# mourisl/Rcorrector

Hardware: AMD Instinct MI355X
Metric: corrected reads/sec (150 bp, k=23) (higher is better)
Workload: dtype u8/int32/u64

## Files before the change

### include/rcorrector_amd.h

```cpp
#ifndef RCORRECTOR_AMD_H
#define RCORRECTOR_AMD_H

#include <stddef.h>
#include <stdint.h>

#ifdef __cplusplus
extern "C" {
#endif

typedef struct rc_ctx rc_ctx;

typedef enum {
    RC_STATUS_OK = 0,
    RC_STATUS_ARG = -1,
    RC_STATUS_HIP = -2,
    RC_STATUS_IO = -3,
    RC_STATUS_STATE = -4,
    RC_STATUS_NOMEM = -5,
    RC_STATUS_NOSPACE = -6
} rc_status;

typedef struct {
    int device;
    int k;
// ... 124 lines not shown
    const char *qual;
    const uint32_t *off;
    char *seq2;
    const char *qual2;
    const uint32_t *off2;
    int32_t *ret, *l, *m, *h;
} rc_batch;
int rc_correct_batch(rc_ctx *ctx, rc_batch *b);

#define RC_MAX_SLOTS 4
int rc_set_slot_lanes(rc_ctx *ctx, int on);
int rc_runtime_prepare(int hw_queues);
int rc_submit(rc_ctx *ctx, const rc_batch *b, int slot);
int rc_wait(rc_ctx *ctx, int slot);
int rc_host_alloc(rc_ctx *ctx, size_t bytes, void **out);
int rc_host_free(rc_ctx *ctx, void *p);
int rc_host_register(void *p, size_t bytes);
int rc_host_unregister(void *p);

typedef struct {
    int mode;
    size_t n;
    uint64_t nbytes;
    const uint32_t *off;
    const uint32_t *bases;
    const uint8_t *qual_bits;
    const uint32_t *exc_pos;
    const uint8_t *exc_chr;
    size_t n_exc;
    int32_t *ret, *l, *m, *h;
    uint32_t *fix_pos;
    uint8_t *fix_chr;
    size_t fix_cap;
    size_t n_fix;
} rc_packed_batch;
size_t rc_pack_bases(const char *seq, size_t begin, size_t end, uint32_t *bases, uint32_t *exc_pos, uint8_t *exc_chr, size_t exc_cap);
int rc_submit_packed(rc_ctx *ctx, rc_packed_batch *b, int slot);
int rc_wait_packed(rc_ctx *ctx, int slot);
void rc_apply_fixes(char *seq, const uint32_t *fix_pos, const uint8_t *fix_chr, size_t n_fix);

typedef struct {
    int mode;
    size_t n;
    int arena_a, arena_b;
    uint64_t begin_a, bytes_a;
    uint64_t begin_b, bytes_b;
    const uint32_t *off;
    const uint8_t *qual_bits;
    int32_t *ret, *l, *m, *h;
    uint32_t *fix_pos;
    uint8_t *fix_chr;
    size_t fix_cap;
    size_t n_fix;
} rc_resident_batch;
int rc_submit_resident(rc_ctx *ctx, rc_resident_batch *b, int slot);
int rc_wait_resident(rc_ctx *ctx, int slot);

#define RC_TRACE_ITER_WORDS 36
typedef struct {
    int32_t max_iter;
    int32_t *counts_before, *counts_after;
    int32_t *flags, *n_iter;
    int32_t *iter;
} rc_trace;
int rc_correct_batch_traced(rc_ctx *ctx, rc_batch *b, rc_trace *t);

typedef struct {
    int mode;
    uint32_t n_reads;
    uint64_t nbytes;
    int32_t max_read_len;
    uint8_t *d_seq;
    const uint8_t *d_qual;
    const uint32_t *d_off;
    int32_t *d_ret, *d_l, *d_m, *d_h;
} rc_device_batch;
int rc_correct_device(rc_ctx *ctx, const rc_device_batch *b);
int rc_strong_threshold_device(rc_ctx *ctx, const uint8_t *d_seq, const uint32_t *d_off, uint32_t n_reads,
                               uint64_t nbytes, int32_t max_read_len, int32_t *d_strong);
int rc_strong_threshold_read(rc_ctx *ctx, const char *seq, int32_t *strong);
int rc_correct_read(rc_ctx *ctx, char *seq, const char *qual, int32_t pair_strong_threshold, int32_t *ret);
int rc_kmer_info_read(rc_ctx *ctx, const char *seq, int32_t *l, int32_t *m, int32_t *h);
int rc_probe_device(rc_ctx *ctx, const uint8_t *d_seq, uint64_t nbytes, int32_t *d_counts);
int rc_sync(rc_ctx *ctx);

int rc_profile_enable(rc_ctx *ctx, int on);
int rc_profile_correct_counters(rc_ctx *ctx, uint64_t *reads_listed, uint64_t *gather_rounds, uint64_t *bucket_requests);
int rc_profile_read_rounds(rc_ctx *ctx, int32_t *d_rounds);
int rc_profile_get(rc_ctx *ctx, int kernel, double *total_ms, uint64_t *launches);
int rc_profile_reset(rc_ctx *ctx);

int rc_selftest_get_bound(rc_ctx *ctx, const int32_t *c, size_t n, double error_rate, int32_t *out_int, double *out_dbl);

int rc_debug_routes(rc_ctx *ctx, uint8_t *cls_out, uint8_t *cand_out, uint64_t *runs_out, uint32_t n);

int rc_summary(const rc_ctx *ctx, uint64_t *total_reads, uint64_t *total_corrections);

#ifdef __cplusplus
}
#endif
#endif
```

### rcorrector_amd/binding.py

```python
import ctypes as C
import os
import subprocess

import numpy as np

HERE = os.path.dirname(os.path.abspath(__file__))
CSRC = os.path.join(HERE, "csrc")

ABI_SYMBOLS = [
    "rc_create", "rc_destroy", "rc_last_error", "rc_device_numa_node", "rc_device_memory",
    "rc_table_build", "rc_table_build_device", "rc_table_load_jfdump",
    "rc_table_count_begin", "rc_table_count_add", "rc_table_count_add_device", "rc_table_count_finish",
    "rc_table_count_keep", "rc_table_count_arenas", "rc_table_count_release", "rc_table_count_park", "rc_table_count_finish_sharded", "rc_submit_resident", "rc_wait_resident",
    "rc_table_count_reads_device", "rc_table_write_jfdump", "rc_table_share", "rc_table_replicate", "rc_table_replicate_async", "rc_table_lookup", "rc_table_export", "rc_table_digest", "rc_table_layout", "rc_table_stats",
    "rc_table_count_spectrum", "rc_table_spectrum",
    "rc_recount_begin", "rc_recount_add", "rc_recount_add_device", "rc_recount_follow", "rc_recount_finish",
    "rc_change_report_begin", "rc_change_report_get", "rc_change_report_end",
    "rc_weak_profile_device", "rc_weak_profile_into",
    "rc_dup_census_begin", "rc_dup_census_get", "rc_dup_census_end", "rc_read_keys_device", "rc_dup_census_merge",
    "rc_trust_profile_device", "rc_trust_profile_begin", "rc_trust_profile_get", "rc_trust_profile_end",
    "rc_mate_overlap_device", "rc_mate_overlap_begin", "rc_mate_overlap_get", "rc_mate_overlap_end",
    "rc_estimate_error_rate", "rc_bad_quality_from_hist", "rc_set_run_params", "rc_set_quality_bits", "rc_pack_quality_bits",
    "rc_correct_batch", "rc_set_slot_lanes", "rc_runtime_prepare", "rc_submit", "rc_wait", "rc_host_alloc", "rc_host_free", "rc_host_register", "rc_host_unregister", "rc_correct_batch_traced", "rc_correct_device", "rc_strong_threshold_device", "rc_probe_device", "rc_sync",
    "rc_strong_threshold_read", "rc_correct_read", "rc_kmer_info_read",
    "rc_pack_bases", "rc_submit_packed", "rc_wait_packed", "rc_apply_fixes",
    "rc_profile_enable", "rc_profile_get", "rc_profile_reset", "rc_profile_correct_counters", "rc_profile_read_rounds", "rc_selftest_get_bound", "rc_debug_routes", "rc_summary",
]


class RcorrectorError(RuntimeError):
    pass


def library_path():
    return os.environ.get("RC_LIB") or os.path.join(HERE, "librcorrector_amd.so")


def build_library(quiet=True):
    subprocess.run(["make", "-C", CSRC, "-j4", "all"], check=True,
                   stdout=subprocess.DEVNULL if quiet else None)
    return library_path()


class _Config(C.Structure):
    _fields_ = [("device", C.c_int), ("k", C.c_int), ("max_fix_per_k", C.c_int)]


class _Batch(C.Structure):
    _fields_ = [("mode", C.c_int), ("n", C.c_size_t),
                ("seq", C.c_void_p), ("qual", C.c_void_p), ("off", C.c_void_p),
                ("seq2", C.c_void_p), ("qual2", C.c_void_p), ("off2", C.c_void_p),
                ("ret", C.c_void_p), ("l", C.c_void_p), ("m", C.c_void_p), ("h", C.c_void_p)]


class _PackedBatch(C.Structure):
    _fields_ = [("mode", C.c_int), ("n", C.c_size_t), ("nbytes", C.c_uint64),
                ("off", C.c_void_p), ("bases", C.c_void_p), ("qual_bits", C.c_void_p),
                ("exc_pos", C.c_void_p), ("exc_chr", C.c_void_p), ("n_exc", C.c_size_t),
                ("ret", C.c_void_p), ("l", C.c_void_p), ("m", C.c_void_p), ("h", C.c_void_p),
                ("fix_pos", C.c_void_p), ("fix_chr", C.c_void_p), ("fix_cap", C.c_size_t), ("n_fix", C.c_size_t)]


class _ResidentBatch(C.Structure):
    _fields_ = [("mode", C.c_int), ("n", C.c_size_t), ("arena_a", C.c_int), ("arena_b", C.c_int),
                ("begin_a", C.c_uint64), ("bytes_a", C.c_uint64), ("begin_b", C.c_uint64), ("bytes_b", C.c_uint64),
                ("off", C.c_void_p), ("qual_bits", C.c_void_p),
                ("ret", C.c_void_p), ("l", C.c_void_p), ("m", C.c_void_p), ("h", C.c_void_p),
                ("fix_pos", C.c_void_p), ("fix_chr", C.c_void_p), ("fix_cap", C.c_size_t), ("n_fix", C.c_size_t)]


class _SpectrumStats(C.Structure):
    _fields_ = [("distinct", C.c_uint64), ("total", C.c_uint64), ("unique", C.c_uint64), ("max_count", C.c_uint64)]


class _RecountStats(C.Structure):
    _fields_ = [("all", _SpectrumStats), ("absent_distinct", C.c_uint64), ("absent_total", C.c_uint64)]


REPORT_MAX_LEN = 1024
REPORT_MAX_PER_READ = 64


class _ChangeReport(C.Structure):
    _fields_ = [("reads", C.c_uint64 * 2), ("reads_changed", C.c_uint64 * 2), ("reads_unfixable", C.c_uint64 * 2), ("changes", C.c_uint64 * 2),
                ("len_hist", C.c_uint64 * REPORT_MAX_LEN * 2), ("by_pos5", C.c_uint64 * REPORT_MAX_LEN * 2), ("by_pos3", C.c_uint64 * REPORT_MAX_LEN * 2),
                ("subst", C.c_uint64 * 4 * 5), ("by_qual", C.c_uint64 * 3), ("per_read", C.c_uint64 * (REPORT_MAX_PER_READ + 1))]


class _ReadWeak(C.Structure):
    _fields_ = [("weak", C.c_int32), ("bad_prefix", C.c_int32), ("bad_suffix", C.c_int32), ("uncovered", C.c_int32)]


class _DupCensus(C.Structure):
    _fields_ = [("units", C.c_uint64), ("distinct_before", C.c_uint64), ("distinct_after", C.c_uint64),
                ("copies_before", C.c_void_p), ("copies_after", C.c_void_p)]


TRUST_MAX_LEN = 1024
_TrustArray = (C.c_uint64 * TRUST_MAX_LEN) * 2
TRUST_FIELDS = ("windows", "solid5", "weak5", "solid3", "weak3")


class _TrustCounts(C.Structure):
    _fields_ = [(n, _TrustArray) for n in TRUST_FIELDS]


# ... 49 lines not shown
            "g.build()' or make -C rcorrector_amd/csrc).  There is no CPU fallback." % path)
    try:
        import torch
    except Exception:
        pass
    try:
        L = C.CDLL(path)
    except OSError as e:
        raise RcorrectorError("cannot load %s: %s" % (path, e))
    vp, sz = C.c_void_p, C.c_size_t
    L.rc_create.restype = vp
    L.rc_create.argtypes = [C.POINTER(_Config), C.c_char_p, sz]
    L.rc_destroy.argtypes = [vp]
    L.rc_last_error.restype = C.c_char_p
    L.rc_last_error.argtypes = [vp]
    L.rc_table_build.argtypes = [vp, vp, vp, sz]
    L.rc_table_build_device.argtypes = [vp, vp, vp, sz]
    L.rc_table_load_jfdump.argtypes = [vp, C.c_char_p, C.POINTER(C.c_int64)]
    L.rc_table_count_reads_device.argtypes = [vp, vp, sz, C.c_int, C.POINTER(C.c_int64)]
    L.rc_table_count_begin.argtypes = [vp]
    L.rc_table_count_add.argtypes = [vp, vp, sz]
    L.rc_table_count_add_device.argtypes = [vp, vp, sz]
    L.rc_table_count_finish.argtypes = [vp, C.c_int, C.POINTER(C.c_int64)]
    L.rc_table_count_keep.argtypes = [vp, C.c_int]
    L.rc_table_count_arenas.argtypes = [vp, C.POINTER(C.c_size_t), vp, sz]
    L.rc_table_count_release.argtypes = [vp]
    L.rc_table_count_park.argtypes = [vp]
    L.rc_table_count_finish_sharded.argtypes = [C.POINTER(C.c_void_p), C.c_int, C.c_int, C.POINTER(C.c_int64)]
    L.rc_set_slot_lanes.argtypes = [vp, C.c_int]
    if hasattr(L, "rc_runtime_prepare"):
        L.rc_runtime_prepare.argtypes = [C.c_int]
    L.rc_submit_resident.argtypes = [vp, C.POINTER(_ResidentBatch), C.c_int]
    L.rc_wait_resident.argtypes = [vp, C.c_int]
    L.rc_table_write_jfdump.argtypes = [vp, C.c_char_p, C.POINTER(C.c_int64)]
    L.rc_table_share.argtypes = [vp, vp]
    L.rc_table_replicate.argtypes = [vp, vp]
    L.rc_table_replicate_async.argtypes = [vp, vp]
    L.rc_device_numa_node.argtypes = [vp]
    L.rc_device_memory.argtypes = [vp, C.POINTER(C.c_uint64), C.POINTER(C.c_uint64)]
    L.rc_table_lookup.argtypes = [vp, vp, sz, vp]
    L.rc_table_export.argtypes = [vp, vp, vp, sz, C.POINTER(C.c_size_t)]
    L.rc_table_digest.argtypes = [vp, C.POINTER(C.c_uint64)]
    L.rc_table_layout.argtypes = [vp]
    L.rc_table_stats.argtypes = [vp, C.POINTER(C.c_uint64), C.POINTER(C.c_uint64), C.POINTER(C.c_uint64)]
    L.rc_table_count_spectrum.argtypes = [vp, C.c_uint32]
    L.rc_table_spectrum.argtypes = [vp, C.c_int, vp, C.c_uint32, C.POINTER(_SpectrumStats)]
    L.rc_recount_begin.argtypes = [vp, C.c_uint32]
    L.rc_recount_add.argtypes = [vp, vp, C.c_size_t]
    L.rc_recount_add_device.argtypes = [vp, vp, C.c_size_t]
    L.rc_recount_follow.argtypes = [vp, C.c_int]
    L.rc_recount_finish.argtypes = [vp, vp, C.POINTER(_RecountStats)]
    L.rc_change_report_begin.argtypes = [vp]
    L.rc_change_report_get.argtypes = [vp, C.POINTER(_ChangeReport)]
    L.rc_change_report_end.argtypes = [vp]
    L.rc_weak_profile_device.argtypes = [vp, vp, vp, C.c_uint32, C.c_uint64, C.c_int32, C.c_int32, vp]
    L.rc_weak_profile_into.argtypes = [vp, C.c_int, vp, C.c_int32]
    L.rc_dup_census_begin.argtypes = [vp]
    L.rc_dup_census_get.argtypes = [vp, C.c_uint32, C.POINTER(_DupCensus)]
    L.rc_dup_census_end.argtypes = [vp]
    L.rc_read_keys_device.argtypes = [vp, vp, vp, C.c_uint32, C.c_uint64, C.c_int, vp]
    L.rc_dup_census_merge.argtypes = [vp, vp]
    L.rc_trust_profile_device.argtypes = [vp, vp, vp, C.c_uint32, C.c_uint64, C.c_int32, C.c_int32, C.c_int32, vp]
    L.rc_trust_profile_begin.argtypes = [vp, C.c_int32]
    L.rc_trust_profile_get.argtypes = [vp, C.POINTER(_TrustProfile)]
    L.rc_trust_profile_end.argtypes = [vp]
    L.rc_mate_overlap_device.argtypes = [vp, vp, vp, vp, C.c_uint32, C.c_uint64, C.c_int32, C.c_int32, C.c_int32, C.c_int32, vp]
    L.rc_mate_overlap_begin.argtypes = [vp, C.c_int32, C.c_int32]
    L.rc_mate_overlap_get.argtypes = [vp, C.POINTER(_MateOverlap)]
    L.rc_mate_overlap_end.argtypes = [vp]
    L.rc_estimate_error_rate.argtypes = [vp, C.c_double, C.POINTER(C.c_double)]
    L.rc_bad_quality_from_hist.restype = C.c_char
    L.rc_bad_quality_from_hist.argtypes = [vp, vp, C.c_int32]
    L.rc_set_run_params.argtypes = [vp, C.c_double, C.c_char]
    L.rc_set_quality_bits.argtypes = [vp, C.c_int]
    L.rc_pack_quality_bits.restype = None
    L.rc_pack_quality_bits.argtypes = [vp, sz, C.c_char, vp]
    L.rc_correct_batch.argtypes = [vp, C.POINTER(_Batch)]
    L.rc_submit.argtypes = [vp, C.POINTER(_Batch), C.c_int]
    L.rc_wait.argtypes = [vp, C.c_int]
    L.rc_host_alloc.argtypes = [vp, sz, C.POINTER(C.c_void_p)]
    L.rc_host_free.argtypes = [vp, vp]
    L.rc_correct_device.argtypes = [vp, C.POINTER(_DeviceBatch)]
    L.rc_probe_device.argtypes = [vp, vp, C.c_uint64, vp]
    L.rc_strong_threshold_device.argtypes = [vp, vp, vp, C.c_uint32, C.c_uint64, C.c_int32, vp]
    L.rc_sync.argtypes = [vp]
    L.rc_strong_threshold_read.argtypes = [vp, C.c_char_p, C.POINTER(C.c_int32)]
    L.rc_correct_read.argtypes = [vp, C.c_char_p, C.c_char_p, C.c_int32, C.POINTER(C.c_int32)]
    L.rc_kmer_info_read.argtypes = [vp, C.c_char_p, C.POINTER(C.c_int32), C.POINTER(C.c_int32), C.POINTER(C.c_int32)]
    L.rc_pack_bases.restype = sz
    L.rc_pack_bases.argtypes = [vp, sz, sz, vp, vp, vp, sz]
    L.rc_submit_packed.argtypes = [vp, C.POINTER(_PackedBatch), C.c_int]
    L.rc_wait_packed.argtypes = [vp, C.c_int]
    L.rc_apply_fixes.restype = None
    L.rc_apply_fixes.argtypes = [vp, vp, vp, sz]
    L.rc_profile_enable.argtypes = [vp, C.c_int]
    L.rc_profile_get.argtypes = [vp, C.c_int, C.POINTER(C.c_double), C.POINTER(C.c_uint64)]
    L.rc_profile_reset.argtypes = [vp]
    L.rc_profile_correct_counters.argtypes = [vp, C.POINTER(C.c_uint64), C.POINTER(C.c_uint64), C.POINTER(C.c_uint64)]
    L.rc_profile_read_rounds.argtypes = [vp, vp]
    L.rc_selftest_get_bound.argtypes = [vp, vp, sz, C.c_double, vp, vp]
    L.rc_debug_routes.argtypes = [vp, vp, vp, vp, C.c_uint32]
    L.rc_summary.argtypes = [vp, C.POINTER(C.c_uint64), C.POINTER(C.c_uint64)]
    _lib = L
    return L


def runtime_prepare(hw_queues=16):
    return load_library().rc_runtime_prepare(int(hw_queues))


def pack_reads(seqs):
    lens = np.fromiter((len(s) for s in seqs), dtype=np.int64, count=len(seqs))
    off = np.zeros(len(seqs) + 1, dtype=np.uint32)
    np.cumsum(lens + 1, out=off[1:])
    if seqs:
        arena = np.frombuffer(b"\0".join(seqs) + b"\0", dtype=np.uint8).copy()
    else:
        arena = np.zeros(0, np.uint8)
    return arena, off


def unpack_reads(arena, off):
    b = arena.tobytes()
    return [b[off[i]:off[i + 1] - 1] for i in range(len(off) - 1)]


def _ptr(x):
    if x is None:
        return None
    if isinstance(x, int):
        return x
    if isinstance(x, np.ndarray):
        return x.ctypes.data
    if hasattr(x, "data_ptr"):
        if getattr(x, "is_cuda", False):
            import torch
            torch.cuda.current_stream(x.device).synchronize()
        return x.data_ptr()
    raise TypeError("cannot take a pointer of %r" % type(x))


class Context:

    def __init__(self, k=23, max_fix_per_k=4, device=0):
        self._L = load_library()
        cfg = _Config(device, k, max_fix_per_k)
        err = C.create_string_buffer(512)
        self._h = self._L.rc_create(C.byref(cfg), err, 512)
        if not self._h:
            raise RcorrectorError(err.value.decode() or "rc_create failed")
        self.k = k

    def close(self):
        if getattr(self, "_h", None):
            for p in getattr(self, "_pinned", []):
                self._L.rc_host_free(self._h, p)
            self._pinned = []
            self._L.rc_destroy(self._h)
            self._h = None

    def __del__(self):
        try:
            self.close()
        except Exception:
            pass

# ... 325 lines not shown

    def count_park(self):
        self._ck(self._L.rc_table_count_park(self._h))

    def count_finish_sharded(self, others, min_count=2):
        hs = (C.c_void_p * (1 + len(others)))(self._h, *[o._h for o in others])
        n = C.c_int64(0)
        self._ck(self._L.rc_table_count_finish_sharded(hs, 1 + len(others), min_count, C.byref(n)))
        return n.value

    def count_release(self):
        self._ck(self._L.rc_table_count_release(self._h))

    def submit_resident(self, slot, mode, off, qual_bits, arena_a, begin_a, bytes_a, arena_b=0, begin_b=0, bytes_b=0, res=None, fix_pos=None,
                        fix_chr=None, fix_cap=None):
        off = np.ascontiguousarray(off, dtype=np.uint32)
        total = len(off) - 1
        if res is None:
            res = [np.zeros(total, dtype=np.int32) for _ in range(4)]
        if fix_pos is None:
            fix_cap = int(bytes_a + bytes_b) if fix_cap is None else fix_cap
            fix_pos, fix_chr = np.zeros(fix_cap, dtype=np.uint32), np.zeros(fix_cap, dtype=np.uint8)
        b = _ResidentBatch()
        b.mode, b.n = mode, (total // 2 if mode == 1 else total)
        b.arena_a, b.begin_a, b.bytes_a = int(arena_a), int(begin_a), int(bytes_a)
        b.arena_b, b.begin_b, b.bytes_b = int(arena_b), int(begin_b), int(bytes_b)
        b.off = off.ctypes.data
        b.qual_bits = None if qual_bits is None else qual_bits.ctypes.data
        b.ret, b.l, b.m, b.h = (r.ctypes.data for r in res)
        b.fix_pos, b.fix_chr, b.fix_cap = fix_pos.ctypes.data, fix_chr.ctypes.data, len(fix_pos)
        self._ck(self._L.rc_submit_resident(self._h, C.byref(b), slot))
        if not hasattr(self, "_inflight_resident"):
            self._inflight_resident = {}
        self._inflight_resident[slot] = (b, res, fix_pos, fix_chr, (off, qual_bits))

    def wait_resident(self, slot):
        self._ck(self._L.rc_wait_resident(self._h, slot))
        b, res, fix_pos, fix_chr, _keep = self._inflight_resident.pop(slot)
        return tuple(res) + (fix_pos[:b.n_fix], fix_chr[:b.n_fix])

    def apply_fixes(self, arena, fix_pos, fix_chr):
        arena = self._arena(arena, "arena")
        fp, fc = np.ascontiguousarray(fix_pos, dtype=np.uint32), np.ascontiguousarray(fix_chr, dtype=np.uint8)
        self._L.rc_apply_fixes(arena.ctypes.data, fp.ctypes.data, fc.ctypes.data, len(fp))

    def host_array(self, n, dtype=np.uint8):
        dt = np.dtype(dtype)
        p = C.c_void_p(0)
        self._ck(self._L.rc_host_alloc(self._h, max(1, n * dt.itemsize), C.byref(p)))
        if not hasattr(self, "_pinned"):
            self._pinned = []
        self._pinned.append(p.value)
        buf = (C.c_uint8 * (n * dt.itemsize)).from_address(p.value)
        return np.frombuffer(buf, dtype=dt, count=n)


    def correct_device(self, mode, n_reads, nbytes, max_read_len, d_seq, d_qual, d_off, d_ret, d_l, d_m, d_h):
        b = _DeviceBatch(mode, n_reads, nbytes, max_read_len, _ptr(d_seq), _ptr(d_qual), _ptr(d_off),
                         _ptr(d_ret), _ptr(d_l), _ptr(d_m), _ptr(d_h))
        self._ck(self._L.rc_correct_device(self._h, C.byref(b)))

    def strong_threshold_device(self, d_seq, d_off, n_reads, nbytes, max_read_len, d_strong):
        self._ck(self._L.rc_strong_threshold_device(self._h, _ptr(d_seq), _ptr(d_off), n_reads, nbytes, max_read_len, _ptr(d_strong)))

    def strong_threshold_read(self, seq):
        out = C.c_int32(0)
        self._ck(self._L.rc_strong_threshold_read(self._h, bytes(seq), C.byref(out)))
        return out.value

    def correct_read(self, seq, qual, pair_strong_threshold=-1):
        buf = C.create_string_buffer(bytes(seq))
        out = C.c_int32(0)
        self._ck(self._L.rc_correct_read(self._h, buf, None if qual is None else bytes(qual), int(pair_strong_threshold), C.byref(out)))
        return out.value, buf.value

    def kmer_info_read(self, seq):
        l, m, h = C.c_int32(0), C.c_int32(0), C.c_int32(0)
        self._ck(self._L.rc_kmer_info_read(self._h, bytes(seq), C.byref(l), C.byref(m), C.byref(h)))
        return l.value, m.value, h.value

    def probe_device(self, d_seq, nbytes, d_counts):
        self._ck(self._L.rc_probe_device(self._h, _ptr(d_seq), nbytes, _ptr(d_counts)))

    def sync(self):
        self._ck(self._L.rc_sync(self._h))

    def profile(self, on=True):
        self._ck(self._L.rc_profile_enable(self._h, int(on)))

    def profile_correct_counters(self):
        a, b, c = C.c_uint64(0), C.c_uint64(0), C.c_uint64(0)
        self._ck(self._L.rc_profile_correct_counters(self._h, C.byref(a), C.byref(b), C.byref(c)))
        return a.value, b.value, c.value

    def profile_read_rounds(self, d_rounds=None):
        self._ck(self._L.rc_profile_read_rounds(self._h, None if d_rounds is None else d_rounds.data_ptr()))

    def profile_reset(self):
        self._ck(self._L.rc_profile_reset(self._h))

    def profile_get(self, kernel):
        ms, n = C.c_double(0), C.c_uint64(0)
        self._ck(self._L.rc_profile_get(self._h, kernel, C.byref(ms), C.byref(n)))
        return ms.value, n.value

    def selftest_get_bound(self, c, error_rate):
        c = np.ascontiguousarray(c, dtype=np.int32)
        oi = np.zeros(len(c), dtype=np.int32)
        od = np.zeros(len(c), dtype=np.float64)
        self._ck(self._L.rc_selftest_get_bound(self._h, c.ctypes.data, len(c), error_rate, oi.ctypes.data, od.ctypes.data))
        return oi, od

    def debug_routes(self, n):
        cls, cand, runs = np.zeros(n, np.uint8), np.zeros(n, np.uint8), np.zeros(n, np.uint64)
        self._ck(self._L.rc_debug_routes(self._h, cls.ctypes.data, cand.ctypes.data, runs.ctypes.data, n))
        return cls, cand, runs

    def summary(self):
        a, b = C.c_uint64(0), C.c_uint64(0)
        self._ck(self._L.rc_summary(self._h, C.byref(a), C.byref(b)))
        return a.value, b.value
```

### rcorrector_amd/csrc/rc_table.hip

```cpp
#include <cstring>
#include <vector>

#include <algorithm>
#include <vector>
#include <rocprim/rocprim.hpp>

#include <chrono>
#include "rc_internal.h"
#include "rc_device.h"

__global__ void k_home_and_index(const uint64_t *__restrict__ canon, uint32_t *__restrict__ home,
                                 uint32_t *__restrict__ idx, size_t n, uint32_t nb_home, int layout, int k, int ext)
{
    size_t j = (size_t)blockIdx.x * blockDim.x + threadIdx.x;
    if (j >= n) return;
    size_t i = n - 1 - j;
    uint32_t h, rem, xrem;
    if (layout)
        rc_packed_addr(canon[i], k, nb_home, ext, &h, &rem, &xrem);
    else
        h = rc_home(canon[i], nb_home);
    home[j] = h;
    idx[j] = (uint32_t)i;
}

__global__ void k_slot_seed(const uint32_t *__restrict__ home_sorted, long long *__restrict__ q, size_t n, int slots)
{
    size_t j = (size_t)blockIdx.x * blockDim.x + threadIdx.x;
    if (j >= n) return;
    q[j] = (long long)slots * home_sorted[j] - (long long)j;
}

__global__ void k_packed_feasible(const uint32_t *__restrict__ home_sorted, const long long *__restrict__ qmax,
                                  const int32_t *__restrict__ counts, size_t n, int ext, unsigned *__restrict__ flags)
{
    size_t j = (size_t)blockIdx.x * blockDim.x + threadIdx.x;
    if (j >= n) return;
    const long long p = qmax[j] + (long long)j;
    if ((uint32_t)counts[j] >= (RC_PACKED_COUNT_MASK >> ext)) atomicAdd(flags + 1, 1u);
    if ((uint32_t)(p / RC_PACKED_SLOTS) - home_sorted[j] > RC_PACKED_MAX_DISP) atomicOr(flags, 2u);
}

__global__ void k_collect_overflow(const uint64_t *__restrict__ canon, const int32_t *__restrict__ counts, size_t n, uint32_t cmask,
                                   unsigned *__restrict__ n_out, uint4 *__restrict__ out, uint32_t *__restrict__ out_idx)
{
    size_t i = (size_t)blockIdx.x * blockDim.x + threadIdx.x;
    if (i >= n || (uint32_t)counts[i] < cmask) return;
    const unsigned o = atomicAdd(n_out, 1u);
    if (o >= RC_PACKED_OVF_MAX) return;
    out[o] = make_uint4((uint32_t)canon[i], (uint32_t)(canon[i] >> 32), (uint32_t)counts[i], 0u);
    out_idx[o] = (uint32_t)i;
}

__global__ void k_scatter(const uint32_t *__restrict__ home_sorted, const uint32_t *__restrict__ idx_sorted,
                          const long long *__restrict__ qmax, const uint64_t *__restrict__ canon,
                          const int32_t *__restrict__ counts, uint32_t *__restrict__ buckets, size_t n, uint32_t nb_home, int layout, int k, int ext)
{
    size_t j = (size_t)blockIdx.x * blockDim.x + threadIdx.x;
    if (j >= n) return;
    const long long p = qmax[j] + (long long)j;
    const int S = rc_layout_slots(layout);
    const uint32_t b = (uint32_t)(p / S), s = (uint32_t)(p % S);
    const uint32_t i = idx_sorted[j];
    const uint64_t key = canon[i];
    if (layout) {
        uint32_t h, rem, xrem;
        rc_packed_addr(key, k, nb_home, ext, &h, &rem, &xrem);
        uint32_t *w = buckets + (size_t)b * RC_BUCKET_DWORDS + s * 2;
        w[0] = rem;
        atomicAnd(w + 1, 0x80000000u);
        const uint32_t cmask = RC_PACKED_COUNT_MASK >> ext, cnt = (uint32_t)counts[i] < cmask ? (uint32_t)counts[i] : cmask;
        atomicOr(w + 1, cnt | (xrem << (27 - ext)) | ((b - h) << 27));
        if (s == 0 && h < b) atomicOr(buckets + (size_t)(b - 1) * RC_BUCKET_DWORDS + (RC_BUCKET_DWORDS - 1), 0x80000000u);
    } else {
        uint32_t *w = buckets + (size_t)b * RC_BUCKET_DWORDS + s * 3;
        w[0] = (uint32_t)key;
        w[1] = (uint32_t)(key >> 32);
        w[2] = (uint32_t)counts[i];
        if (s == 0 && home_sorted[j] < b) buckets[(size_t)(b - 1) * RC_BUCKET_DWORDS + (RC_BUCKET_DWORDS - 1)] = 1u;
    }
}

__global__ void k_filter_set(const uint64_t *__restrict__ canon, size_t n, uint32_t nb_home, int k, int ext, uint32_t *__restrict__ filter, uint32_t words,
                             int kind)
{
    size_t i = (size_t)blockIdx.x * blockDim.x + threadIdx.x;
    if (i >= n) return;
    if (kind) {
        const uint64_t x = canon[i], rv = rc_revcomp(x, k);
        uint32_t w, m;
// ... 685 lines not shown
                const int f = (int)((w[q >> 2] >> (8 * (q & 3))) & 0xffu);
                if (i0 + q < n && f) {
#pragma unroll
                    for (int c = 0; c < NS; ++c) mine += f == first + c * step ? (1ull << (16 * c)) : 0ull;
                }
            }
        }
        uint64_t inc = mine;
#pragma unroll
        for (int o = 1; o < 64; o <<= 1) {
            const uint64_t y = __shfl_up(inc, o, 64);
            inc += lane >= (uint32_t)o ? y : 0ull;
        }
        if (lane == 63) s_wave[wave] = inc;
        __syncthreads();
        uint64_t before = 0, total = 0;
#pragma unroll
        for (int q = 0; q < 4; ++q) {
            before += (uint32_t)q < wave ? s_wave[q] : 0ull;
            total += s_wave[q];
        }
        if (total) {
            if (t < (uint32_t)NS) {
                const uint32_t c = (uint32_t)((total >> (16 * t)) & 0xffffu);
                s_base[t] = c ? atomicAdd(count + t, c) : 0u;
            }
            __syncthreads();
            if (mine) {
                const uint64_t ex = before + inc - mine;
                uint32_t pos[NS];
#pragma unroll
                for (int c = 0; c < NS; ++c) pos[c] = s_base[c] + (uint32_t)((ex >> (16 * c)) & 0xffffu);
#pragma unroll
                for (int q = 0; q < 16; ++q) {
                    const int f = (int)((w[q >> 2] >> (8 * (q & 3))) & 0xffu);
                    if (i0 + q < n && f) {
#pragma unroll
                        for (int c = 0; c < NS; ++c)
                            if (f == first + c * step) list[(size_t)c * stride + pos[c]++] = values ? values[i0 + (uint32_t)q] : i0 + (uint32_t)q;
                    }
                }
            }
        }
        __syncthreads();
    }
}

template <int NS>
static int rc_compact_sections(rc_ctx *ctx, const uint8_t *d_flag, uint32_t n, int first, int step, uint32_t *d_list, size_t stride, uint32_t *d_count,
                               const uint32_t *d_values = nullptr)
{
    RC_CHECK_HIP(ctx, hipMemsetAsync(d_count, 0, NS * sizeof(uint32_t), ctx->stream));
    if (n == 0) return RC_OK;
    unsigned grid = (n + 4095u) / 4096u;
    if (grid > (unsigned)ctx->n_cu * 32u) grid = (unsigned)ctx->n_cu * 32u;
    hipLaunchKernelGGL(k_compact_sections<NS>, dim3(grid), dim3(256), 0, ctx->stream, d_flag, n, first, step, d_list, stride, d_count, d_values);
    RC_CHECK_HIP(ctx, hipGetLastError());
    return RC_OK;
}

int rc_launch_compact(rc_ctx *ctx, const uint8_t *d_cls, uint32_t n, uint32_t *d_list, size_t stride, uint32_t *d_count)
{
    return rc_compact_sections<RC_WORK_CLASSES>(ctx, d_cls, n, RC_WORK_CLASSES, -1, d_list, stride, d_count);
}

__global__ __launch_bounds__(256) void k_gather_u8(const uint8_t *__restrict__ src, const uint32_t *__restrict__ idx, uint32_t n, uint8_t *__restrict__ dst)
{
    const uint32_t i = blockIdx.x * 256u + threadIdx.x;
    if (i < n) dst[i] = src[idx[i]];
}
int rc_launch_compact_local(rc_ctx *ctx, const uint8_t *d_cls, uint32_t n, uint32_t *d_list, size_t stride, uint32_t *d_count)
{
    int rc = rc_dbuf_reserve(ctx, &ctx->tier_flag, (size_t)n + 256);
    if (rc) return rc;
    hipLaunchKernelGGL(k_gather_u8, dim3((n + 255) / 256), dim3(256), 0, ctx->stream, d_cls, (const uint32_t *)ctx->loc_list.p, n, (uint8_t *)ctx->tier_flag.p);
    return rc_compact_sections<RC_WORK_CLASSES>(ctx, (const uint8_t *)ctx->tier_flag.p, n, RC_WORK_CLASSES, -1, d_list, stride, d_count, (const uint32_t *)ctx->loc_list.p);
}

int rc_launch_compact_flag(rc_ctx *ctx, const uint8_t *d_flag, uint32_t n, uint32_t *d_list, size_t stride, uint32_t *d_count)
{
    return rc_compact_sections<3>(ctx, d_flag, n, 1, 1, d_list, stride, d_count);
}

#define RC_KEY_TILE 40960
__global__ __launch_bounds__(256) void k_unit_key(const uint8_t *__restrict__ seq, size_t nbytes, const uint32_t *__restrict__ off,
                                                  uint32_t n_units, int mode, int k, uint32_t units_per_block,
                                                  uint32_t *__restrict__ keys, uint32_t *__restrict__ idx)
{
    __shared__ __attribute__((aligned(16))) uint8_t s_raw[RC_KEY_TILE + 48];
    const uint32_t u0 = blockIdx.x * units_per_block;
    if (u0 >= n_units) return;
    const uint32_t nu = n_units - u0 < units_per_block ? n_units - u0 : units_per_block;
    const uint32_t r0 = mode == 2 ? 2u * u0 : u0, r1 = mode == 2 ? 2u * (u0 + nu) : u0 + nu;
    const size_t b0 = off[r0], b1 = off[r1], a0 = b0 & ~(size_t)15;
    for (size_t c = threadIdx.x; a0 + 16 * c < b1; c += 256) {
        const size_t g = a0 + 16 * c;
        uint4 v = make_uint4(0, 0, 0, 0);
        if (g + 16 <= nbytes) {
            v = *reinterpret_cast<const uint4 *>(seq + g);
        } else {
            uint32_t w[4] = {0, 0, 0, 0};
            for (size_t q = 0; g + q < nbytes; ++q) w[q >> 2] |= (uint32_t)seq[g + q] << (8 * (q & 3));
            v = make_uint4(w[0], w[1], w[2], w[3]);
        }
        *reinterpret_cast<uint4 *>(s_raw + 16 * c) = v;
    }
    __syncthreads();
    if (threadIdx.x >= nu) return;
    const uint32_t u = u0 + threadIdx.x;
    const uint32_t r = mode == 2 ? 2u * u : u;
    const uint32_t o = (uint32_t)(off[r] - a0);
    const int len = (int)(off[r + 1] - off[r]) - 1;
#ifndef RC_KEY_KMER
    const int m = k < 16 ? k : 16;
    const uint32_t mask = m == 16 ? 0xFFFFFFFFu : ((1u << (2 * m)) - 1u);
    const int top = 2 * (m - 1);
    uint32_t fw = 0, rv = 0, best = 0xFFFFFFFFu;
    int valid = 0;
#ifdef RC_KEY_OFFSET
    int best_i = 0;
    bool best_rev = false;
#endif
    for (int i = 0; i < len; ++i) {
        const uint32_t c = s_raw[o + i];
        const uint32_t b = ((c >> 1) ^ (c >> 2)) & 3u;
        const uint32_t d = c - 65u;
        const bool acgt = d < 20u && ((0x80045u >> d) & 1u);
        valid = acgt ? valid + 1 : 0;
        fw = ((fw << 2) | b) & mask;
        rv = (rv >> 2) | ((3u - b) << top);
        if (valid >= m) {
            uint32_t h = (fw < rv ? fw : rv) * 0x9E3779B1u;
            h ^= h >> 15;
            h *= 0x2C1B3C6Du;
            h ^= h >> 13;
#ifdef RC_KEY_OFFSET
            if (h < best) {
                best_i = i;
                best_rev = rv < fw;
            }
#endif
            best = h < best ? h : best;
        }
    }
#ifdef RC_KEY_OFFSET
    if (best != 0xFFFFFFFFu) {
        int p = best_rev ? len - 1 - best_i : best_i - m + 1;
        p = (p >> 1) > 127 ? 127 : (p >> 1);
        best = (best & ~0x7Fu) | (uint32_t)(127 - p);
    }
#endif
#else
    const uint64_t mask = rc_kmer_mask(k);
    uint64_t fw = 0, rv = 0;
    uint32_t best = 0xFFFFFFFFu;
    int valid = 0;
    for (int i = 0; i < len; ++i) {
        const uint32_t c = s_raw[o + i];
        int b = -1;
        b = c == 'A' ? 0 : b;
        b = c == 'C' ? 1 : b;
        b = c == 'G' ? 2 : b;
        b = c == 'T' ? 3 : b;
        valid = b < 0 ? 0 : valid + 1;
        fw = ((fw << 2) | (uint64_t)(b & 3)) & mask;
        rv = (rv >> 2) | ((uint64_t)(3 - (b & 3)) << (2 * (k - 1)));
        if (valid >= k) {
            const uint32_t h = rc_hash(fw < rv ? fw : rv);
            best = h < best ? h : best;
        }
    }
#endif
    keys[u] = best;
    idx[u] = u;
}

__global__ void k_probe_order(const uint32_t *__restrict__ unit_sorted, uint32_t n, int mode, uint32_t *__restrict__ list,
                              const uint32_t *__restrict__ off, uint2 *__restrict__ span)
{
    const uint32_t i = blockIdx.x * blockDim.x + threadIdx.x;
    if (i >= n) return;
    uint32_t r;
    if (mode == 1)
        r = unit_sorted[i >> 1] + ((i & 1u) ? (n >> 1) : 0u);
    else if (mode == 2)
        r = 2u * unit_sorted[i >> 1] + (i & 1u);
    else
        r = unit_sorted[i];
    list[i] = r;
    const uint32_t g0 = off[r];
    span[i] = make_uint2(g0, off[r + 1] - g0);
}

int rc_launch_locality_order(rc_ctx *ctx, const rc_device_batch_args &a, size_t nbytes)
{
    const uint32_t n = a.n, n_units = a.mode ? n >> 1 : n;
    int rc;
    if ((rc = rc_dbuf_reserve(ctx, &ctx->loc_a, (size_t)n_units * 16 + 256))) return rc;
    if ((rc = rc_dbuf_reserve(ctx, &ctx->loc_list, (size_t)n * 4 + 256))) return rc;
    if ((rc = rc_dbuf_reserve(ctx, &ctx->loc_span, (size_t)n * 8 + 256))) return rc;
    uint32_t *keys = (uint32_t *)ctx->loc_a.p, *keys2 = keys + n_units, *idx = keys2 + n_units, *idx2 = idx + n_units;
    uint32_t upb = (uint32_t)(RC_KEY_TILE / ((size_t)(a.max_len + 1) * (a.mode == 2 ? 2 : 1)));
    if (upb > 256) upb = 256;
    if (upb < 1) upb = 1;
    hipLaunchKernelGGL(k_unit_key, dim3((n_units + upb - 1) / upb), dim3(256), 0, ctx->stream, a.seq, nbytes, a.off, n_units, a.mode, ctx->k, upb, keys, idx);
    size_t t1 = 0;
    RC_CHECK_HIP(ctx, rocprim::radix_sort_pairs(nullptr, t1, keys, keys2, idx, idx2, (size_t)n_units, 0, 32, ctx->stream));
    if ((rc = rc_dbuf_reserve(ctx, &ctx->sel_tmp, t1))) return rc;
    RC_CHECK_HIP(ctx, rocprim::radix_sort_pairs(ctx->sel_tmp.p, t1, keys, keys2, idx, idx2, (size_t)n_units, 0, 32, ctx->stream));
    hipLaunchKernelGGL(k_probe_order, dim3((n + 255) / 256), dim3(256), 0, ctx->stream, idx2, n, a.mode, (uint32_t *)ctx->loc_list.p, a.off,
                       (uint2 *)ctx->loc_span.p);
    RC_CHECK_HIP(ctx, hipGetLastError());
    return RC_OK;
}

__global__ __launch_bounds__(256) void k_tier_flags(const uint32_t *__restrict__ off, const uint32_t *__restrict__ list, uint32_t n, int mode,
                                                    int s_hi, int m_hi, uint8_t *__restrict__ flag)
{
    const uint32_t i = blockIdx.x * 256u + threadIdx.x;
    if (i >= n) return;
    const uint32_t r = list[i];
    int ml = (int)(off[r + 1] - off[r]) - 1;
    if (mode != 0) {
        const uint32_t half = n >> 1, mr = mode == 1 ? (r < half ? r + half : r - half) : (r ^ 1u);
        const int m1 = (int)(off[mr + 1] - off[mr]) - 1;
        ml = m1 > ml ? m1 : ml;
    }
    flag[i] = ml <= s_hi ? 0 : (ml <= m_hi ? 1 : 2);
}

int rc_launch_tier_lists(rc_ctx *ctx, const rc_device_batch_args &a, int s_hi, int m_hi)
{
    int rc;
    const size_t stride = ((size_t)a.n + 63) & ~(size_t)63;
    if ((rc = rc_dbuf_reserve(ctx, &ctx->tier_flag, (size_t)a.n + 256))) return rc;
    if ((rc = rc_dbuf_reserve(ctx, &ctx->tier_list, stride * 2 * 4 + 256))) return rc;
    ctx->tier_stride = stride;
    hipLaunchKernelGGL(k_tier_flags, dim3((a.n + 255) / 256), dim3(256), 0, ctx->stream, a.off, (const uint32_t *)ctx->loc_list.p, a.n, a.mode, s_hi, m_hi,
                       (uint8_t *)ctx->tier_flag.p);
    RC_CHECK_HIP(ctx, hipGetLastError());
    return rc_compact_sections<2>(ctx, (const uint8_t *)ctx->tier_flag.p, a.n, 1, 1, (uint32_t *)ctx->tier_list.p, stride,
                                  (uint32_t *)((char *)ctx->work.p + RC_WORK_NTIER_OFF), (const uint32_t *)ctx->loc_list.p);
}

template <bool EXT>
__global__ __launch_bounds__(RC_PROBE_THREADS) void k_probe(rc_table_view T, const uint8_t *__restrict__ seq,
                                                            size_t nbytes, int k, int32_t *__restrict__ counts)
{
    __shared__ uint32_t s_code[RC_PROBE_TILE / 16 + 4];
    __shared__ uint16_t s_inv[RC_PROBE_TILE / 16 + 4];
    __shared__ uint16_t s_nul[RC_PROBE_TILE / 16 + 4];
    const size_t tile0 = (size_t)blockIdx.x * RC_PROBE_TILE;
    const int t = threadIdx.x;

    rc_tile_stage(seq, 0, nbytes, tile0, s_code, s_inv, s_nul);
    __syncthreads();
    const uint32_t *m_inv = reinterpret_cast<const uint32_t *>(s_inv);
    const uint32_t *m_nul = reinterpret_cast<const uint32_t *>(s_nul);

#pragma unroll 2
    for (int a = t; a < RC_PROBE_TILE; a += RC_PROBE_THREADS) {
        const size_t g = tile0 + (size_t)a;
        if (g + (size_t)k > nbytes) break;
        const rc_tile_win w = rc_tile_window(s_code, m_inv, m_nul, a, k);
        if (w.nul) continue;
        const int cnt = w.bad ? 0 : rc_table_lookup<EXT>(T, rc_canonical(w.code, k));
        __builtin_nontemporal_store(cnt, &counts[g]);
    }
}

template <bool EXT>
__global__ __launch_bounds__(RC_PROBE_THREADS) void k_probe_list(rc_table_view T, const uint8_t *__restrict__ seq, size_t nbytes,
                                                                 const uint32_t *__restrict__ off, const uint32_t *__restrict__ list,
                                                                 uint32_t n, uint32_t reads_per_block, int k, int32_t *__restrict__ counts,
                                                                 int mode, int skip_hi, const uint32_t *__restrict__ n_list)
{
    __shared__ __attribute__((aligned(16))) uint32_t s_raw[(RC_PROBE_TILE + 64) / 4];
    __shared__ uint32_t s_code[RC_PROBE_TILE / 16 + 4];
    __shared__ uint16_t s_inv[RC_PROBE_TILE / 16 + 4];
    __shared__ uint16_t s_nul[RC_PROBE_TILE / 16 + 4];
    __shared__ uint32_t s_lpos[RC_PLIST_MAX_READS + 1], s_gpos[RC_PLIST_MAX_READS], s_len1[RC_PLIST_MAX_READS];
    const int t = threadIdx.x;
    const uint32_t n_eff = n_list ? *n_list : n;
    for (uint32_t i0 = blockIdx.x * reads_per_block; i0 < n_eff; i0 += gridDim.x * reads_per_block) {
    const uint32_t nr = n_eff - i0 < reads_per_block ? n_eff - i0 : reads_per_block;
    bool any_live = false;
    if ((uint32_t)t < nr) {
        const uint32_t r = list[i0 + t], g0 = off[r];
        uint32_t len1 = off[r + 1] - g0;
        if (skip_hi >= 0) {
            uint32_t ml1 = len1;
            if (mode != 0) {
                const uint32_t half = n >> 1, mr = mode == 1 ? (r < half ? r + half : r - half) : (r ^ 1u);
                const uint32_t m1 = off[mr + 1] - off[mr];
// ... 107 lines not shown
```

Before: 360.0 million.

## Rewrite unit-key minimizer kernel with 2-bit packed tiles and lane-parallel windows

```diff
diff --git a/include/rcorrector_amd.h b/include/rcorrector_amd.h
--- a/include/rcorrector_amd.h
+++ b/include/rcorrector_amd.h
@@ -230,6 +230,8 @@
 int rc_correct_read(rc_ctx *ctx, char *seq, const char *qual, int32_t pair_strong_threshold, int32_t *ret);
 int rc_kmer_info_read(rc_ctx *ctx, const char *seq, int32_t *l, int32_t *m, int32_t *h);
 int rc_probe_device(rc_ctx *ctx, const uint8_t *d_seq, uint64_t nbytes, int32_t *d_counts);
+int rc_unit_keys_device(rc_ctx *ctx, int mode, uint32_t n_reads, uint64_t nbytes, int32_t max_read_len, const uint8_t *d_seq,
+                        const uint32_t *d_off, uint32_t *d_keys);
 int rc_sync(rc_ctx *ctx);
 
 int rc_profile_enable(rc_ctx *ctx, int on);
diff --git a/rcorrector_amd/binding.py b/rcorrector_amd/binding.py
--- a/rcorrector_amd/binding.py
+++ b/rcorrector_amd/binding.py
@@ -21,7 +21,7 @@
     "rc_trust_profile_device", "rc_trust_profile_begin", "rc_trust_profile_get", "rc_trust_profile_end",
     "rc_mate_overlap_device", "rc_mate_overlap_begin", "rc_mate_overlap_get", "rc_mate_overlap_end",
     "rc_estimate_error_rate", "rc_bad_quality_from_hist", "rc_set_run_params", "rc_set_quality_bits", "rc_pack_quality_bits",
-    "rc_correct_batch", "rc_set_slot_lanes", "rc_runtime_prepare", "rc_submit", "rc_wait", "rc_host_alloc", "rc_host_free", "rc_host_register", "rc_host_unregister", "rc_correct_batch_traced", "rc_correct_device", "rc_strong_threshold_device", "rc_probe_device", "rc_sync",
+    "rc_correct_batch", "rc_set_slot_lanes", "rc_runtime_prepare", "rc_submit", "rc_wait", "rc_host_alloc", "rc_host_free", "rc_host_register", "rc_host_unregister", "rc_correct_batch_traced", "rc_correct_device", "rc_strong_threshold_device", "rc_probe_device", "rc_unit_keys_device", "rc_sync",
     "rc_strong_threshold_read", "rc_correct_read", "rc_kmer_info_read",
     "rc_pack_bases", "rc_submit_packed", "rc_wait_packed", "rc_apply_fixes",
     "rc_profile_enable", "rc_profile_get", "rc_profile_reset", "rc_profile_correct_counters", "rc_profile_read_rounds", "rc_selftest_get_bound", "rc_debug_routes", "rc_summary",
@@ -237,6 +237,7 @@
     L.rc_host_free.argtypes = [vp, vp]
     L.rc_correct_device.argtypes = [vp, C.POINTER(_DeviceBatch)]
     L.rc_probe_device.argtypes = [vp, vp, C.c_uint64, vp]
+    L.rc_unit_keys_device.argtypes = [vp, C.c_int, C.c_uint32, C.c_uint64, C.c_int32, vp, vp, vp]
     L.rc_strong_threshold_device.argtypes = [vp, vp, vp, C.c_uint32, C.c_uint64, C.c_int32, vp]
     L.rc_sync.argtypes = [vp]
     L.rc_strong_threshold_read.argtypes = [vp, C.c_char_p, C.POINTER(C.c_int32)]
@@ -728,6 +729,9 @@
     def probe_device(self, d_seq, nbytes, d_counts):
         self._ck(self._L.rc_probe_device(self._h, _ptr(d_seq), nbytes, _ptr(d_counts)))
 
+    def unit_keys_device(self, mode, n_reads, nbytes, max_read_len, d_seq, d_off, d_keys):
+        self._ck(self._L.rc_unit_keys_device(self._h, int(mode), n_reads, nbytes, max_read_len, _ptr(d_seq), _ptr(d_off), _ptr(d_keys)))
+
     def sync(self):
         self._ck(self._L.rc_sync(self._h))
 
diff --git a/rcorrector_amd/csrc/rc_table.hip b/rcorrector_amd/csrc/rc_table.hip
--- a/rcorrector_amd/csrc/rc_table.hip
+++ b/rcorrector_amd/csrc/rc_table.hip
@@ -6,6 +6,7 @@
 #include <rocprim/rocprim.hpp>
 
 #include <chrono>
+#include "../../include/rcorrector_amd.h"
 #include "rc_internal.h"
 #include "rc_device.h"
 
@@ -857,97 +858,107 @@
     return rc_compact_sections<3>(ctx, d_flag, n, 1, 1, d_list, stride, d_count);
 }
 
-#define RC_KEY_TILE 40960
+#define RC_KEY_TILE 16384
+constexpr int RC_KEY_LANES = 16;
+template <bool M16>
 __global__ __launch_bounds__(256) void k_unit_key(const uint8_t *__restrict__ seq, size_t nbytes, const uint32_t *__restrict__ off,
                                                   uint32_t n_units, int mode, int k, uint32_t units_per_block,
                                                   uint32_t *__restrict__ keys, uint32_t *__restrict__ idx)
 {
-    __shared__ __attribute__((aligned(16))) uint8_t s_raw[RC_KEY_TILE + 48];
+    constexpr int G = RC_KEY_LANES, V = 16 / G, NCH = RC_KEY_TILE / 16 + 1;
+    static_assert(G * V == 16 && 256 % G == 0, "RC_KEY_LANES divides 16");
+    __shared__ uint32_t s_code[NCH + 2];
+    __shared__ uint16_t s_bad[NCH + 2];
     const uint32_t u0 = blockIdx.x * units_per_block;
     if (u0 >= n_units) return;
     const uint32_t nu = n_units - u0 < units_per_block ? n_units - u0 : units_per_block;
     const uint32_t r0 = mode == 2 ? 2u * u0 : u0, r1 = mode == 2 ? 2u * (u0 + nu) : u0 + nu;
     const size_t b0 = off[r0], b1 = off[r1], a0 = b0 & ~(size_t)15;
-    for (size_t c = threadIdx.x; a0 + 16 * c < b1; c += 256) {
-        const size_t g = a0 + 16 * c;
-        uint4 v = make_uint4(0, 0, 0, 0);
-        if (g + 16 <= nbytes) {
-            v = *reinterpret_cast<const uint4 *>(seq + g);
-        } else {
+    const size_t nch = (b1 - a0 + 15) >> 4;
+    const bool fits = b1 >= b0 && nch <= (size_t)NCH;
+    if (fits) {
+        for (size_t c = threadIdx.x; c < nch; c += 256) {
+            const size_t g = a0 + 16 * c;
             uint32_t w[4] = {0, 0, 0, 0};
-            for (size_t q = 0; g + q < nbytes; ++q) w[q >> 2] |= (uint32_t)seq[g + q] << (8 * (q & 3));
-            v = make_uint4(w[0], w[1], w[2], w[3]);
-        }
-        *reinterpret_cast<uint4 *>(s_raw + 16 * c) = v;
+            if (g + 16 <= nbytes) {
+                const uint4 v = *reinterpret_cast<const uint4 *>(seq + g);
+                w[0] = v.x, w[1] = v.y, w[2] = v.z, w[3] = v.w;
+            } else {
+                for (size_t q = 0; g + q < nbytes; ++q) w[q >> 2] |= (uint32_t)seq[g + q] << (8 * (q & 3));
+            }
+            uint32_t code, am, tm, bad;
+            rc_pack16m(w, code, am, tm, bad);
+            s_code[c + 1] = code;
+            s_bad[c + 1] = (uint16_t)bad;
+        }
+        if (threadIdx.x < 2) {
+            const size_t e = threadIdx.x ? nch + 1 : 0;
+            s_code[e] = 0;
+            s_bad[e] = 0xFFFFu;
+        }
     }
     __syncthreads();
-    if (threadIdx.x >= nu) return;
-    const uint32_t u = u0 + threadIdx.x;
-    const uint32_t r = mode == 2 ? 2u * u : u;
-    const uint32_t o = (uint32_t)(off[r] - a0);
-    const int len = (int)(off[r + 1] - off[r]) - 1;
-#ifndef RC_KEY_KMER
-    const int m = k < 16 ? k : 16;
-    const uint32_t mask = m == 16 ? 0xFFFFFFFFu : ((1u << (2 * m)) - 1u);
-    const int top = 2 * (m - 1);
-    uint32_t fw = 0, rv = 0, best = 0xFFFFFFFFu;
-    int valid = 0;
-#ifdef RC_KEY_OFFSET
-    int best_i = 0;
-    bool best_rev = false;
-#endif
-    for (int i = 0; i < len; ++i) {
-        const uint32_t c = s_raw[o + i];
-        const uint32_t b = ((c >> 1) ^ (c >> 2)) & 3u;
-        const uint32_t d = c - 65u;
-        const bool acgt = d < 20u && ((0x80045u >> d) & 1u);
-        valid = acgt ? valid + 1 : 0;
-        fw = ((fw << 2) | b) & mask;
-        rv = (rv >> 2) | ((3u - b) << top);
-        if (valid >= m) {
-            uint32_t h = (fw < rv ? fw : rv) * 0x9E3779B1u;
-            h ^= h >> 15;
-            h *= 0x2C1B3C6Du;
-            h ^= h >> 13;
-#ifdef RC_KEY_OFFSET
-            if (h < best) {
-                best_i = i;
-                best_rev = rv < fw;
+    const int m = M16 ? 16 : k;
+    const uint32_t kmask = M16 ? 0xFFFFFFFFu : ((1u << (2 * m)) - 1u), mmask = (1u << m) - 1u, down = 32u - 2u * (uint32_t)m;
+    const uint32_t g = threadIdx.x & (G - 1);
+    for (uint32_t ub = 0; ub < nu; ub += 256 / G) {
+        const uint32_t ul = ub + threadIdx.x / G;
+        const bool live = ul < nu;
+        const uint32_t u = u0 + ul;
+        uint32_t o = 0;
+        int nwin = 0;
+        if (live && fits) {
+            const uint32_t r = mode == 2 ? 2u * u : u;
+            const uint32_t g0 = off[r];
+            o = g0 - (uint32_t)a0;
+            nwin = (int)(off[r + 1] - g0) - 1 - m + 1;
+        }
+        uint32_t cp[V], mp[V], wi[V], sh[V], qs[V], best = 0xFFFFFFFFu;
+#pragma unroll
+        for (int v = 0; v < V; ++v) {
+            const uint32_t a = o + g + (uint32_t)(G * v), q = a & 15u;
+            wi[v] = (a >> 4) + (q ? 1u : 0u);
+            sh[v] = (32u - 2u * q) & 31u;
+            qs[v] = q ? q : 16u;
+            cp[v] = mp[v] = 0;
+            if ((int)g + G * v < nwin) {
+                cp[v] = s_code[wi[v]];
+                mp[v] = s_bad[wi[v]];
             }
-#endif
-            best = h < best ? h : best;
-        }
-    }
-#ifdef RC_KEY_OFFSET
-    if (best != 0xFFFFFFFFu) {
-        int p = best_rev ? len - 1 - best_i : best_i - m + 1;
-        p = (p >> 1) > 127 ? 127 : (p >> 1);
-        best = (best & ~0x7Fu) | (uint32_t)(127 - p);
-    }
-#endif
-#else
-    const uint64_t mask = rc_kmer_mask(k);
-    uint64_t fw = 0, rv = 0;
-    uint32_t best = 0xFFFFFFFFu;
-    int valid = 0;
-    for (int i = 0; i < len; ++i) {
-        const uint32_t c = s_raw[o + i];
-        int b = -1;
-        b = c == 'A' ? 0 : b;
-        b = c == 'C' ? 1 : b;
-        b = c == 'G' ? 2 : b;
-        b = c == 'T' ? 3 : b;
-        valid = b < 0 ? 0 : valid + 1;
-        fw = ((fw << 2) | (uint64_t)(b & 3)) & mask;
-        rv = (rv >> 2) | ((uint64_t)(3 - (b & 3)) << (2 * (k - 1)));
-        if (valid >= k) {
-            const uint32_t h = rc_hash(fw < rv ? fw : rv);
-            best = h < best ? h : best;
-        }
-    }
-#endif
-    keys[u] = best;
-    idx[u] = u;
+        }
+        for (int p = (int)g; p < nwin; p += 16) {
+#pragma unroll
+            for (int v = 0; v < V; ++v) {
+                if (p + G * v < nwin) {
+                    ++wi[v];
+                    const uint32_t cn = s_code[wi[v]], mn = s_bad[wi[v]];
+                    const uint32_t x = __builtin_amdgcn_alignbit(cp[v], cn, sh[v]);
+                    const uint32_t inv = ((mp[v] | (mn << 16)) >> qs[v]) & mmask;
+                    const uint32_t fw = M16 ? x : x >> down;
+                    uint32_t rv = rc_brev32(x);
+                    rv = ((rv & 0x55555555u) << 1) | ((rv >> 1) & 0x55555555u);
+                    rv = ~rv & kmask;
+                    uint32_t h = (fw < rv ? fw : rv) * 0x9E3779B1u;
+                    h ^= h >> 15;
+                    h *= 0x2C1B3C6Du;
+                    h ^= h >> 13;
+                    h = inv ? 0xFFFFFFFFu : h;
+                    best = h < best ? h : best;
+                    cp[v] = cn;
+                    mp[v] = mn;
+                }
+            }
+        }
+#pragma unroll
+        for (int d = G / 2; d >= 1; d >>= 1) {
+            const uint32_t other = (uint32_t)__shfl_xor((int)best, d, 64);
+            best = other < best ? other : best;
+        }
+        if (live && g == 0) {
+            keys[u] = best;
+            if (idx) idx[u] = u;
+        }
+    }
 }
 
 __global__ void k_probe_order(const uint32_t *__restrict__ unit_sorted, uint32_t n, int mode, uint32_t *__restrict__ list,
@@ -967,6 +978,19 @@
     span[i] = make_uint2(g0, off[r + 1] - g0);
 }
 
+static void rc_launch_unit_key(rc_ctx *ctx, const uint8_t *seq, size_t nbytes, const uint32_t *off, uint32_t n_units, int mode, int max_len,
+                               uint32_t *keys, uint32_t *idx)
+{
+    if (!n_units) return;
+    uint32_t upb = (uint32_t)(RC_KEY_TILE / ((size_t)(max_len > 0 ? max_len + 1 : 1) * (mode == 2 ? 2 : 1)));
+    if (upb < 1) upb = 1;
+    const dim3 grid((n_units + upb - 1) / upb);
+    if (ctx->k >= 16)
+        hipLaunchKernelGGL(k_unit_key<true>, grid, dim3(256), 0, ctx->stream, seq, nbytes, off, n_units, mode, ctx->k, upb, keys, idx);
+    else
+        hipLaunchKernelGGL(k_unit_key<false>, grid, dim3(256), 0, ctx->stream, seq, nbytes, off, n_units, mode, ctx->k, upb, keys, idx);
+}
+
 int rc_launch_locality_order(rc_ctx *ctx, const rc_device_batch_args &a, size_t nbytes)
 {
     const uint32_t n = a.n, n_units = a.mode ? n >> 1 : n;
@@ -975,16 +999,47 @@
     if ((rc = rc_dbuf_reserve(ctx, &ctx->loc_list, (size_t)n * 4 + 256))) return rc;
     if ((rc = rc_dbuf_reserve(ctx, &ctx->loc_span, (size_t)n * 8 + 256))) return rc;
     uint32_t *keys = (uint32_t *)ctx->loc_a.p, *keys2 = keys + n_units, *idx = keys2 + n_units, *idx2 = idx + n_units;
-    uint32_t upb = (uint32_t)(RC_KEY_TILE / ((size_t)(a.max_len + 1) * (a.mode == 2 ? 2 : 1)));
-    if (upb > 256) upb = 256;
-    if (upb < 1) upb = 1;
-    hipLaunchKernelGGL(k_unit_key, dim3((n_units + upb - 1) / upb), dim3(256), 0, ctx->stream, a.seq, nbytes, a.off, n_units, a.mode, ctx->k, upb, keys, idx);
+    rc_launch_unit_key(ctx, a.seq, nbytes, a.off, n_units, a.mode, a.max_len, keys, idx);
     size_t t1 = 0;
     RC_CHECK_HIP(ctx, rocprim::radix_sort_pairs(nullptr, t1, keys, keys2, idx, idx2, (size_t)n_units, 0, 32, ctx->stream));
     if ((rc = rc_dbuf_reserve(ctx, &ctx->sel_tmp, t1))) return rc;
     RC_CHECK_HIP(ctx, rocprim::radix_sort_pairs(ctx->sel_tmp.p, t1, keys, keys2, idx, idx2, (size_t)n_units, 0, 32, ctx->stream));
     hipLaunchKernelGGL(k_probe_order, dim3((n + 255) / 256), dim3(256), 0, ctx->stream, idx2, n, a.mode, (uint32_t *)ctx->loc_list.p, a.off,
                        (uint2 *)ctx->loc_span.p);
+    RC_CHECK_HIP(ctx, hipGetLastError());
+    return RC_OK;
+}
+
+int rc_unit_keys_device(rc_ctx *ctx, int mode, uint32_t n_reads, uint64_t nbytes, int32_t max_read_len, const uint8_t *d_seq, const uint32_t *d_off,
+                        uint32_t *d_keys)
+{
+    if (!ctx) return RC_ERR_ARG;
+    if (mode < 0 || mode > 2) {
+        rc_set_error(ctx, "unit_keys_device: mode must be 0, 1 or 2 (got %d)", mode);
+        return RC_ERR_ARG;
+    }
+    if (mode != 0 && (n_reads & 1u)) {
+        rc_set_error(ctx, "unit_keys_device: %s mode needs an even number of reads (got %u)", mode == 1 ? "paired" : "interleaved", n_reads);
+        return RC_ERR_ARG;
+    }
+    if (n_reads && (!d_seq || !d_off || !d_keys)) {
+        rc_set_error(ctx, "unit_keys_device: null pointer");
+        return RC_ERR_ARG;
+    }
+    if ((uintptr_t)d_seq & 15u) {
+        rc_set_error(ctx, "unit_keys_device: d_seq must be 16-byte aligned");
+        return RC_ERR_ARG;
+    }
+    if (nbytes >= (1ull << 32)) {
+        rc_set_error(ctx, "unit_keys_device: arena of %llu bytes exceeds the 4 GiB batch limit", (unsigned long long)nbytes);
+        return RC_ERR_ARG;
+    }
+    if (max_read_len < 0 || ((size_t)max_read_len + 1) * (mode == 2 ? 2 : 1) > (size_t)RC_KEY_TILE) {
+        rc_set_error(ctx, "unit_keys_device: max_read_len %d: a unit must fit the key kernel's tile of %d bytes", max_read_len, RC_KEY_TILE);
+        return RC_ERR_ARG;
+    }
+    RC_CHECK_HIP(ctx, hipSetDevice(ctx->device));
+    rc_launch_unit_key(ctx, d_seq, (size_t)nbytes, d_off, mode ? n_reads >> 1 : n_reads, mode, max_read_len, d_keys, nullptr);
     RC_CHECK_HIP(ctx, hipGetLastError());
     return RC_OK;
 }
```

Result: no change. 360.0 million (-0.0%).
